# Orange-OpenSource/pyDcop

Measured on AMD Instinct MI355X. Metric: MaxSum iterations/sec on 100k-var random graph-coloring DCOP, higher is better.
Workload: dtype f64; 1 GPU; coloring_100k; n_vars=100000, n_factors=200000, n_edges=400000, domain=3, params=damping 0.5/both, stability 0.1, start leafs, parallelism=one GPU, 1 launch(es) per cycle, parity_checked=True, parity_test=tests/test_gpu_parity.py::test_north_star_100k_coloring

## Files before the change

### pydcop_amd/csrc/kernels.h

```cpp
#pragma once
#include <hip/hip_runtime.h>

#include <cmath>
#include <cstdint>
#include <cstring>
#include <type_traits>
#include <utility>

#include "layout.h"

namespace mxs {

constexpr int SAME_COUNT = 4;
#ifndef MXS_ASM_MIN
#define MXS_ASM_MIN 1
#endif
#ifndef SWEEP_MIN_WAVES
#define SWEEP_MIN_WAVES 4
#endif

#ifndef MXS_NT
#define MXS_NT 0
#endif
constexpr int NT_STREAMING = 9;
#define MXS_NT_FLAGS(NT)                                                                        \
    constexpr bool NT_IDX = ((NT) & 1) != 0, NT_PREV = ((NT) & 2) != 0, NT_GATHER = ((NT) & 4) != 0; \
    (void)NT_IDX, (void)NT_PREV, (void)NT_GATHER
template <bool NT, typename U>
__device__ __forceinline__ U ldp(const U* p) {
    if constexpr (NT) return __builtin_nontemporal_load(p);
    return *p;
}

template <typename F, int... I>
__device__ __forceinline__ void static_for_impl(F&& f, std::integer_sequence<int, I...>) {
    (f(std::integral_constant<int, I>{}), ...);
}
template <int N, typename F>
__device__ __forceinline__ void static_for(F&& f) {
    static_for_impl(f, std::make_integer_sequence<int, N>{});
}

constexpr int STAGE_BYTES_PER_WAVE = 64 * 2 * MAX_REG_D * 8;
__shared__ double g_stage[BLOCK / 64][STAGE_BYTES_PER_WAVE / 8];

struct Piece16 {
    unsigned int w[4];
};
typedef unsigned int v4u __attribute__((ext_vector_type(4)));
template <bool NT_STORE>
__device__ __forceinline__ void store_piece16(char* dst, const char* src) {
    if constexpr (NT_STORE) {
        __builtin_nontemporal_store(*(const v4u*)__builtin_assume_aligned(src, 16), (v4u*)__builtin_assume_aligned(dst, 16));
        return;
    }
    *(Piece16*)__builtin_assume_aligned(dst, 16) = *(const Piece16*)__builtin_assume_aligned(src, 16);
}
#ifndef MXS_NT_TIGHT
#define MXS_NT_TIGHT 1
#endif

template <typename T, int ELEMS, int NT = MXS_NT>
__device__ __forceinline__ void wave_store_linear(T* arr, int64_t wave_base, const T (&vals)[ELEMS]) {
    constexpr bool NT_STORE = (NT & 8) != 0;
    static_assert(64 * ELEMS * sizeof(T) % 16 == 0 && 64 * ELEMS * sizeof(T) <= STAGE_BYTES_PER_WAVE, "");
    if constexpr (ELEMS * sizeof(T) % 16 != 0) {
        const int w = (int)threadIdx.x >> 6, l = (int)threadIdx.x & 63;
        char* so = (char*)g_stage[w];
        __builtin_amdgcn_wave_barrier();
#pragma unroll
        for (int d = 0; d < ELEMS; ++d) ((T*)so)[l * ELEMS + d] = vals[d];
        __builtin_amdgcn_wave_barrier();
        char* out = (char*)(arr + wave_base);
        constexpr int BYTES = 64 * ELEMS * (int)sizeof(T), FULL = BYTES / 1024, REST = (BYTES % 1024) / 16;
#pragma unroll
        for (int k = 0; k < FULL; ++k) store_piece16<NT_STORE && MXS_NT_TIGHT>(out + k * 1024 + l * 16, so + k * 1024 + l * 16);
        if (REST > 0 && l < REST) store_piece16<NT_STORE && MXS_NT_TIGHT>(out + FULL * 1024 + l * 16, so + FULL * 1024 + l * 16);
        return;
    }
    const int w = (int)threadIdx.x >> 6, l = (int)threadIdx.x & 63;
    char* so = (char*)g_stage[w];
    __builtin_amdgcn_wave_barrier();
#pragma unroll
    for (int d = 0; d < ELEMS; ++d) ((T*)so)[l * ELEMS + d] = vals[d];
    __builtin_amdgcn_wave_barrier();
    char* out = (char*)(arr + wave_base);
    constexpr int PIECES = ELEMS * (int)sizeof(T) / 16;
#pragma unroll
    for (int k = 0; k < PIECES; ++k) store_piece16<NT_STORE>(out + k * 1024 + l * 16, so + k * 1024 + l * 16);
}

template <typename T>
struct SweepArgs {
    const T* v2f_old;
    T* v2f_new;
    const T* f2v_old;
    T* f2v_new;
    const T* tables;
    const uint8_t* ctables;
    int32_t tab_neg;
    const T* var_cost;
    uint8_t* cF;
    uint8_t* cV;
    const int32_t* edge_v2f;
    const int32_t* f2v_off;
    const int32_t* vrowptr;
    const int32_t* vslot_f2v;
    const int32_t* vslot_v2f;
    const int32_t* vell;
    const WaveMeta* vwave;
    const HubBlock* hub_blocks;
    const int32_t* vdom;
    const int64_t* vcost_off;
    const int32_t* init_idx;
    const FactorGen* fgen;
    const int32_t* edge_gen_factor;
    const int32_t* edge_dom;
    int32_t* sel;
    T* belief;
    T damping;
    T stability;
    int32_t damp_f;
    int32_t damp_v;
    int32_t start;
    int32_t start_mode;
    int32_t null_f2v;
    int64_t* timeline;
    uint32_t* halo_flags;
    uint32_t need_epoch;
    T* send_out;
    const int32_t* send_slot;
    int32_t n_peers;
    int32_t me;
    int32_t ghost_lo;
    const T* ghost_old;
    int32_t peer_first[MXS_MAX_PEERS];
    T* peer_dst[MXS_MAX_PEERS];
    int32_t n_classes;
    int32_t block_base[MAX_CLASSES];
    const ClassInfo* classes;
    const uint32_t* sched;
};

template <typename T>
__device__ __forceinline__ T pos_inf() {
    return (T)INFINITY;
}
__device__ __forceinline__ double absT(double x) { return fabs(x); }
__device__ __forceinline__ float absT(float x) { return fabsf(x); }

template <typename T>
__device__ __forceinline__ bool comp_match(T c, T prev_c, T stability) {
    if (prev_c != c) {
        const T delta = absT(prev_c - c);
        if (prev_c + c != (T)0) {
            if (!(((T)2 * delta / absT(prev_c + c)) < stability)) return false;
        } else {
            return false;
        }
    }
    return true;
}

template <typename T, int D>
__device__ __forceinline__ uint8_t damp_and_filter(T (&m)[D], const T (&prev)[D], uint8_t cnt,
                                                   bool damp_on, T damping, T stability) {
    if (cnt > 0 && damp_on) {
#pragma unroll
        for (int d = 0; d < D; ++d) m[d] = damping * prev[d] + ((T)1 - damping) * m[d];
    }
    bool match = cnt > 0;
#pragma unroll
    for (int d = 0; d < D; ++d) match = match && comp_match(m[d], prev[d], stability);
    if (!match) return 1;
    if (cnt < SAME_COUNT) return (uint8_t)(cnt + 1);
#pragma unroll
    for (int d = 0; d < D; ++d) m[d] = prev[d];
    return cnt;
}

template <typename T, int D>
struct Msg {
    static constexpr int H = half_stride(D, (int)sizeof(T));
    static constexpr int ALIGN = (H * (int)sizeof(T)) % 16 == 0 ? 16 : ((H * (int)sizeof(T)) % 8 == 0 ? 8 : 4);
    template <bool NT = false>
    static __device__ __forceinline__ void load(const T* p, T (&m)[D]) {
        const T* q = (const T*)__builtin_assume_aligned(p, ALIGN);
#pragma unroll
        for (int d = 0; d < D; ++d) m[d] = ldp<NT>(q + d);
    }
    static __device__ __forceinline__ void store(T* p, const T (&m)[D]) {
        T* q = (T*)__builtin_assume_aligned(p, ALIGN);
#pragma unroll
        for (int d = 0; d < H; ++d) q[d] = d < D ? m[d < D ? d : 0] : (T)0;
    }
    static __device__ __forceinline__ void load_sys(const T* p, T (&m)[D]) {
#pragma unroll
        for (int d = 0; d < D; ++d) m[d] = __hip_atomic_load(p + d, __ATOMIC_RELAXED, __HIP_MEMORY_SCOPE_SYSTEM);
    }
    static constexpr bool CNT_IN_MSG = H > D;
    template <bool NT = false>
    static __device__ __forceinline__ uint8_t load_c(const T* p, T (&m)[D]) {
        const T* q = (const T*)__builtin_assume_aligned(p, ALIGN);
#pragma unroll
        for (int d = 0; d < D; ++d) m[d] = ldp<NT>(q + d);
        return (uint8_t)(int)ldp<NT>(q + (D < H ? D : 0));
    }
    static __device__ __forceinline__ T padded(const T (&m)[D], uint8_t cnt, int d) {
        return d < D ? m[d < D ? d : 0] : (d == D ? (T)(int)cnt : (T)0);
    }
    static __device__ __forceinline__ void store_c(T* p, const T (&m)[D], uint8_t cnt) {
        T* q = (T*)__builtin_assume_aligned(p, ALIGN);
#pragma unroll
        for (int d = 0; d < H; ++d) q[d] = padded(m, cnt, d);
    }
};

template <typename T, int N, int NT = MXS_NT>
__device__ __forceinline__ void load_table(const SweepArgs<T>& a, const ClassInfo& ci, int j, T (&tab)[N]) {
    MXS_NT_FLAGS(NT);
    if (ci.tab_type == TAB_FULL) {
#pragma unroll
        for (int k = 0; k < N; ++k) tab[k] = ldp<NT_IDX>(a.tables + ci.tab_base + (int64_t)k * ci.count + j);
        return;
    }
    if (ci.tab_type == TAB_I8) {
        constexpr int REC = tab_record_bytes(N, 1);
        uint32_t w[REC / 4];
        const uint32_t* p = (const uint32_t*)__builtin_assume_aligned(
            a.ctables + ci.ctab_base + (int64_t)j * REC, REC >= 16 ? 16 : REC);
#pragma unroll
        for (int i = 0; i < REC / 4; ++i) w[i] = ldp<NT_IDX>(p + i);
#pragma unroll
        for (int k = 0; k < N; ++k) tab[k] = (T)(int)(int8_t)(uint8_t)(w[k >> 2] >> (8 * (k & 3)));
    } else if (ci.tab_type == TAB_I16) {
        constexpr int REC = tab_record_bytes(N, 2);
        uint32_t w[REC / 4];
        const uint32_t* p = (const uint32_t*)__builtin_assume_aligned(
            a.ctables + ci.ctab_base + (int64_t)j * REC, REC >= 16 ? 16 : REC);
#pragma unroll
        for (int i = 0; i < REC / 4; ++i) w[i] = ldp<NT_IDX>(p + i);
#pragma unroll
        for (int k = 0; k < N; ++k) tab[k] = (T)(int)(int16_t)(uint16_t)(w[k >> 1] >> (16 * (k & 1)));
    } else {
        constexpr int REC = tab_record_bytes(N, 4);
        uint32_t w[REC / 4];
        const uint32_t* p = (const uint32_t*)__builtin_assume_aligned(
            a.ctables + ci.ctab_base + (int64_t)j * REC, REC >= 16 ? 16 : REC);
#pragma unroll
        for (int i = 0; i < REC / 4; ++i) w[i] = ldp<NT_IDX>(p + i);
#pragma unroll
        for (int k = 0; k < N; ++k) {
            float f;
            __builtin_memcpy(&f, &w[k], 4);
            tab[k] = (T)f;
        }
    }
    if (a.tab_neg) {
#pragma unroll
        for (int k = 0; k < N; ++k) tab[k] = -tab[k];
    }
}

template <typename T, int D, int NT = MXS_NT>
__device__ __forceinline__ void factor_unary(const SweepArgs<T>& a, const ClassInfo& ci, int j) {
    MXS_NT_FLAGS(NT);
    constexpr int H = Msg<T, D>::H;
    const int64_t fo = ci.f2v_base + (int64_t)j * H;
    const int e = ci.edge_base + j;
    constexpr bool CIM = Msg<T, D>::CNT_IN_MSG;
    T out[D], prev[D], tab[D];
    uint8_t cn;
    if constexpr (CIM) cn = Msg<T, D>::template load_c<NT_PREV>(a.f2v_old + fo, prev);
    else {
        Msg<T, D>::template load<NT_PREV>(a.f2v_old + fo, prev);
        cn = a.cF[e];
    }
    load_table<T, D, NT>(a, ci, j, tab);
#pragma unroll
    for (int d = 0; d < D; ++d)
        out[d] = tab[d] + (T)0;
    uint8_t c = 0;
    if (!a.start)
        c = damp_and_filter<T, D>(out, prev, cn, a.damp_f != 0, a.damping, a.stability);
    if constexpr (CIM) {
        Msg<T, D>::store_c(a.f2v_new + fo, out, c);
    } else {
        Msg<T, D>::store(a.f2v_new + fo, out);
        a.cF[e] = c;
    }
}

template <typename T, int D, bool P2P = false, int NT = MXS_NT, bool CUT_HALF = true>
__device__ __forceinline__ void factor_binary(const SweepArgs<T>& a, const ClassInfo& ci, int j) {
    MXS_NT_FLAGS(NT);
    constexpr int H = Msg<T, D>::H;
    const int e = ci.edge_base + 2 * j;
    const int64_t fo0 = ci.f2v_base + (int64_t)j * H, fo1 = ci.f2v_base1 + (int64_t)j * H;
    constexpr bool CIM = Msg<T, D>::CNT_IN_MSG;
    const bool do0 = !CUT_HALF || ci.own_pos != 2, do1 = !CUT_HALF || ci.own_pos != 1;
    const int v0 = do1 ? ldp<NT_IDX>(a.edge_v2f + e) : 0, v1 = do0 ? ldp<NT_IDX>(a.edge_v2f + e + 1) : 0;
    uint8_t cn0 = 0, cn1 = 0;
    T m0[D], p0[D], m1[D], p1[D], tab[D * D];
#pragma unroll
    for (int d = 0; d < D; ++d) m0[d] = p0[d] = m1[d] = p1[d] = (T)0;
    if constexpr (CIM) {
        if (do0) cn0 = Msg<T, D>::template load_c<NT_PREV>(a.f2v_old + fo0, p0);
        if (do1) cn1 = Msg<T, D>::template load_c<NT_PREV>(a.f2v_old + fo1, p1);
    } else {
        if (do0) {
            cn0 = a.cF[e];
            Msg<T, D>::template load<NT_PREV>(a.f2v_old + fo0, p0);
        }
        if (do1) {
            cn1 = a.cF[e + 1];
            Msg<T, D>::template load<NT_PREV>(a.f2v_old + fo1, p1);
        }
    }
    load_table<T, D * D, NT>(a, ci, j, tab);
    if constexpr (P2P) {
        if (do1) {
            if (v0 >= a.ghost_lo) Msg<T, D>::load_sys(a.ghost_old + (v0 - a.ghost_lo), m0);
            else Msg<T, D>::load(a.v2f_old + v0, m0);
        }
        if (do0) {
            if (v1 >= a.ghost_lo) Msg<T, D>::load_sys(a.ghost_old + (v1 - a.ghost_lo), m1);
            else Msg<T, D>::load(a.v2f_old + v1, m1);
        }
    } else {
        if (do1) Msg<T, D>::template load<NT_GATHER>(a.v2f_old + v0, m0);
        if (do0) Msg<T, D>::template load<NT_GATHER>(a.v2f_old + v1, m1);
    }
    T o0[D], o1[D];
#pragma unroll
    for (int x = 0; x < D; ++x) {
        T best0 = pos_inf<T>(), best1 = pos_inf<T>();
#pragma unroll
        for (int y = 0; y < D; ++y) {
            const T c0 = tab[x * D + y] + ((T)0 + m1[y]);
            if (best0 > c0) best0 = c0;
            const T c1 = tab[y * D + x] + ((T)0 + m0[y]);
            if (best1 > c1) best1 = c1;
        }
        o0[x] = best0;
        o1[x] = best1;
    }
    uint8_t c0 = 0, c1 = 0;
    if (a.start) {
        const bool sends = a.start_mode == MXS_START_ALL;
#pragma unroll
        for (int d = 0; d < D; ++d) {
            o0[d] = sends ? o0[d] : (T)0;
            o1[d] = sends ? o1[d] : (T)0;
        }
    } else {
        c0 = damp_and_filter<T, D>(o0, p0, cn0, a.damp_f != 0, a.damping, a.stability);
        c1 = damp_and_filter<T, D>(o1, p1, cn1, a.damp_f != 0, a.damping, a.stability);
    }
    const int lw = (int)threadIdx.x & 63;
    if constexpr ((64 * H * sizeof(T)) % 16 == 0) {
        if ((j - lw + 63) < ci.count) {
            T full[H];
            if (do0) {
#pragma unroll
                for (int d = 0; d < H; ++d) full[d] = Msg<T, D>::padded(o0, CIM ? c0 : 0, d);
                wave_store_linear<T, H, NT>(a.f2v_new, fo0 - (int64_t)lw * H, full);
            }
            if (do1) {
#pragma unroll
                for (int d = 0; d < H; ++d) full[d] = Msg<T, D>::padded(o1, CIM ? c1 : 0, d);
                wave_store_linear<T, H, NT>(a.f2v_new, fo1 - (int64_t)lw * H, full);
            }
        } else {
            if (do0) Msg<T, D>::store_c(a.f2v_new + fo0, o0, CIM ? c0 : 0);
            if (do1) Msg<T, D>::store_c(a.f2v_new + fo1, o1, CIM ? c1 : 0);
        }
    } else {
        if (do0) Msg<T, D>::store_c(a.f2v_new + fo0, o0, CIM ? c0 : 0);
        if (do1) Msg<T, D>::store_c(a.f2v_new + fo1, o1, CIM ? c1 : 0);
    }
    if constexpr (!CIM) {
        if (do0) a.cF[e] = c0;
        if (do1) a.cF[e + 1] = c1;
    }
}

template <typename T>
__device__ __forceinline__ T factor_gen_value(const SweepArgs<T>& a, const FactorGen& fg, int pos,
                                              int d, int64_t others) {
    T best = pos_inf<T>();
    for (int64_t lin = 0; lin < others; ++lin) {
        int64_t rem = others, l = lin, t = 0;
        T sum_cost = (T)0;
        for (int i = 0; i < fg.arity; ++i) {
            const int e = fg.edge_base + i;
            const int Di = a.edge_dom[e];
            int digit;
            if (i == pos) {
                digit = d;
            } else {
                rem /= Di;
                digit = (int)(l / rem);
                l -= (int64_t)digit * rem;
                sum_cost += a.v2f_old[a.edge_v2f[e] + digit];
            }
            t = t * Di + digit;
        }
        const T cur = a.tables[fg.tab_off + t] + sum_cost;
        if (best > cur) best = cur;
    }
    return best;
}

template <typename T>
__device__ __forceinline__ void factor_generic(const SweepArgs<T>& a, const ClassInfo& ci, int j) {
    const int e = ci.edge_base + j;
    const FactorGen fg = a.fgen[a.edge_gen_factor[e]];
    const int pos = e - fg.edge_base;
    const int D = a.edge_dom[e];
    const T* prev = a.f2v_old + a.f2v_off[e];
    T* w = a.f2v_new + a.f2v_off[e];
    int64_t others = 1;
    for (int i = 0; i < fg.arity; ++i)
        if (i != pos) others *= a.edge_dom[fg.edge_base + i];
    if (a.start) {
        const bool sends = (fg.arity == 1 && a.start_mode != MXS_START_ALL) ||
                           a.start_mode == MXS_START_ALL;
        for (int d = 0; d < D; ++d) w[d] = sends ? factor_gen_value(a, fg, pos, d, others) : (T)0;
        a.cF[e] = 0;
        return;
    }
    const uint8_t cnt = a.cF[e];
    const bool damp = cnt > 0 && a.damp_f;
    bool match = cnt > 0;
    for (int d = 0; d < D; ++d) {
        T m = factor_gen_value(a, fg, pos, d, others);
        const T p = prev[d];
        if (damp) m = a.damping * p + ((T)1 - a.damping) * m;
        if (match) match = comp_match(m, p, a.stability);
        w[d] = m;
    }
    uint8_t out = 1;
    if (match) {
        if (cnt < SAME_COUNT) {
            out = (uint8_t)(cnt + 1);
        } else {
            out = cnt;
            for (int d = 0; d < D; ++d) w[d] = prev[d];
        }
    }
    a.cF[e] = out;
}

template <typename T, int D, bool P2P = false, int NT = MXS_NT>
__device__ __forceinline__ void variable_pack(const SweepArgs<T>& a, const ClassInfo& ci, int item) {
    MXS_NT_FLAGS(NT);
    constexpr int H = Msg<T, D>::H;
    const int lane_id = item + (int)threadIdx.x;
    if (lane_id >= ci.count) return;
    const int64_t pos = ci.ell_base + lane_id;
    const WaveMeta wm = a.vwave[__builtin_amdgcn_readfirstlane((int)(pos >> 6))];
    const uint32_t dn = (uint32_t)wm.deg_nv;
    const int deg = (int)(dn & 255u), nv = (int)((dn >> 8) & 255u);
    const int l = (int)threadIdx.x & 63;
    const int var = (int)(((uint32_t)l * (dn >> 16)) >> 15);
    const int k = l - var * deg;
    const bool has = var < nv;
    const int v = wm.first_var + (has ? var : 0);
    const int32_t slot = ldp<NT_IDX>(a.vell + pos);
    const int32_t send_at = a.send_slot != nullptr ? a.send_slot[pos] : -1;
    constexpr bool CIM = Msg<T, D>::CNT_IN_MSG;
    T pv[D], in[D], c[D], b[D], m[D];
    const int64_t vo = ci.v2f_base + (int64_t)lane_id * H;
    uint8_t cnt;
    if constexpr (CIM) cnt = Msg<T, D>::template load_c<NT_PREV>(a.v2f_old + vo, pv);
    else {
        cnt = a.cV[ci.cv_base + lane_id];
        Msg<T, D>::template load<NT_PREV>(a.v2f_old + vo, pv);
    }
    Msg<T, D>::template load<NT_GATHER>(a.f2v_old + (has ? slot : a.null_f2v), in);
#pragma unroll
    for (int d = 0; d < D; ++d) c[d] = a.var_cost[ci.cost_base + (int64_t)(v - ci.first) * D + d];
    int init = -1;
    if (a.start) init = a.init_idx[v];
    const int seg = l - (has ? k : 0);
    T sum_cost = (T)0;
#pragma unroll
    for (int d = 0; d < D; ++d) {
        T bd = c[d], md = c[d];
        for (int kk = 0; kk < deg; ++kk) {
            const T x = __shfl(in[d], seg + kk, 64);
            bd += x;
            if (kk != k) {
                sum_cost += x;
                md += x;
            }
        }
        b[d] = bd;
        m[d] = md;
    }
    int best = 0;
    T best_c = b[0];
#pragma unroll
    for (int d = 1; d < D; ++d)
        if (b[d] < best_c) {
            best = d;
            best_c = b[d];
        }
    if (init >= 0) {
        best = init;
        best_c = (T)0;
    }
    if (has && k == 0) {
        a.sel[v] = best;
        a.belief[v] = best_c;
    }
    const T avg = sum_cost / (T)D;
#pragma unroll
    for (int d = 0; d < D; ++d) m[d] = m[d] - avg;
    uint8_t co = 0;
    if (a.start) {
        const bool sends = (deg == 1 && a.start_mode == MXS_START_LEAFS) ||
                           a.start_mode != MXS_START_LEAFS;
#pragma unroll
        for (int d = 0; d < D; ++d) m[d] = sends ? m[d] : (T)0;
    } else {
        co = damp_and_filter<T, D>(m, pv, cnt, a.damp_v != 0, a.damping, a.stability);
    }
    if (!has) {
        co = 0;
#pragma unroll
        for (int d = 0; d < D; ++d) m[d] = (T)0;
    }
    if (send_at >= 0) {
        T* dst = a.send_out + (int64_t)send_at * H;
        if constexpr (P2P) {
            T* base = a.peer_dst[0];
            int first = a.peer_first[0];
#pragma unroll
            for (int q = 1; q < MXS_MAX_PEERS; ++q) {
                const bool ge = send_at >= a.peer_first[q];
                base = ge ? a.peer_dst[q] : base;
                first = ge ? a.peer_first[q] : first;
            }
            dst = base + (int64_t)(send_at - first) * H;
        }
        Msg<T, D>::store_c(dst, m, CIM ? co : 0);
    }
    if constexpr ((64 * H * sizeof(T)) % 16 == 0) {
        T full[H];
#pragma unroll
        for (int d = 0; d < H; ++d) full[d] = Msg<T, D>::padded(m, CIM ? co : 0, d);
        wave_store_linear<T, H, NT>(a.v2f_new, vo - (int64_t)l * H, full);
    } else {
        Msg<T, D>::store(a.v2f_new + vo, m);
    }
    if constexpr (!CIM) a.cV[ci.cv_base + lane_id] = co;
}

constexpr int PACK8_D = 8;
template <typename T>
__device__ __forceinline__ void variable_pack8_block(const SweepArgs<T>& a, const ClassInfo& ci, int block) {
    constexpr int H = PACK8_D;
    static_assert(half_stride(5, (int)sizeof(T)) == H && half_stride(8, (int)sizeof(T)) == H, "records of 5..8 values are 8 elements long");
    const int lane_id = block * BLOCK + (int)threadIdx.x;
    if (lane_id >= ci.count) return;
    const int64_t pos = ci.ell_base + lane_id;
    const WaveMeta wm = a.vwave[__builtin_amdgcn_readfirstlane((int)(pos >> 6))];
    const uint32_t dn = (uint32_t)wm.deg_nv;
    const int deg = (int)(dn & 255u), nv = (int)((dn >> 8) & 255u);
    const int l = (int)threadIdx.x & 63;
    const int var = (int)(((uint32_t)l * (dn >> 16)) >> 15);
    const int k = l - var * deg;
    const bool has = var < nv;
    const int v = wm.first_var + (has ? var : 0);
    const int32_t slot = a.vell[pos];
    const int D = ci.uni_D ? ci.uni_D : a.vdom[v];
    const int64_t vo = ci.v2f_base + (int64_t)lane_id * H;
    const uint8_t cnt = a.cV[ci.cv_base + lane_id];
    T pv[H], in[H], c[H], m[H];
    Msg<T, H>::load(a.v2f_old + vo, pv);
    Msg<T, H>::load(a.f2v_old + (has ? slot : a.null_f2v), in);
    const T* cp = a.var_cost + (ci.uni_D ? ci.cost_base + (int64_t)(v - ci.first) * ci.uni_D : a.vcost_off[v]);
#pragma unroll
    for (int d = 0; d < H; ++d) {
        c[d] = d < D ? cp[d < D ? d : 0] : (T)0;
        in[d] = d < D ? in[d] : (T)0;
    }
    int init = -1;
    if (a.start) init = a.init_idx[v];
    const int seg = l - (has ? k : 0);
    T sum_cost = (T)0, best_c = (T)0;
    int best = 0;
    const int DU = ci.uni_D ? ci.uni_D : H;
    static_for<H>([&](auto dc) __attribute__((always_inline)) {
        constexpr int d = decltype(dc)::value;
        T bd = c[d], md = c[d];
        if (d < DU) {
            for (int kk = 0; kk < deg; ++kk) {
                const T x = __shfl(in[d], seg + kk, 64);
                bd += x;
                if (kk != k) {
                    sum_cost += x;
                    md += x;
                }
            }
        }
        m[d] = md;
        if (d == 0 || (d < D && bd < best_c)) {
            best = d;
            best_c = bd;
        }
    });
    if (init >= 0) {
        best = init;
        best_c = (T)0;
    }
    if (has && k == 0) {
        a.sel[v] = best;
        a.belief[v] = best_c;
    }
    const T avg = sum_cost / (T)D;
#pragma unroll
    for (int d = 0; d < H; ++d) m[d] = m[d] - avg;
    uint8_t co = 0;
    if (a.start) {
        const bool sends = (deg == 1 && a.start_mode == MXS_START_LEAFS) || a.start_mode != MXS_START_LEAFS;
#pragma unroll
        for (int d = 0; d < H; ++d) m[d] = sends ? m[d] : (T)0;
    } else {
        if (cnt > 0 && a.damp_v) {
#pragma unroll
            for (int d = 0; d < H; ++d) m[d] = a.damping * pv[d] + ((T)1 - a.damping) * m[d];
        }
        bool match = cnt > 0;
#pragma unroll
        for (int d = 0; d < H; ++d) match = match && (d >= D || comp_match(m[d], pv[d], a.stability));
        if (!match) {
            co = 1;
        } else if (cnt < SAME_COUNT) {
            co = (uint8_t)(cnt + 1);
        } else {
            co = cnt;
#pragma unroll
            for (int d = 0; d < H; ++d) m[d] = pv[d];
        }
    }
#pragma unroll
    for (int d = 0; d < H; ++d) m[d] = (has && d < D) ? m[d] : (T)0;
    if (!has) co = 0;
    wave_store_linear<T, H>(a.v2f_new, vo - (int64_t)l * H, m);
    a.cV[ci.cv_base + lane_id] = co;
}
template <typename T>
__global__ void __launch_bounds__(BLOCK) k_variable_pack8(SweepArgs<T> a, const ClassInfo* __restrict__ cls) {
    const ClassInfo ci = cls[0];
    variable_pack8_block<T>(a, ci, (int)blockIdx.x);
}

template <typename T>
__device__ __forceinline__ void variable_generic(const SweepArgs<T>& a, const ClassInfo& ci, int j) {
    if (ci.start_only && !a.start) return;
    const int v = ci.first + j;
    const int D = a.vdom[v];
    const int k0 = a.vrowptr[v], k1 = a.vrowptr[v + 1];
    const int deg = k1 - k0;
    const T* c = a.var_cost + a.vcost_off[v];
    int best = 0;
    T best_c = (T)0;
    for (int d = 0; d < D; ++d) {
        T b = c[d];
        for (int k = k0; k < k1; ++k) b += a.f2v_old[a.vslot_f2v[k] + d];
        if (d == 0 || b < best_c) {
            best = d;
            best_c = b;
        }
    }
    if (a.start && a.init_idx[v] >= 0) {
        best = a.init_idx[v];
        best_c = (T)0;
    }
    a.sel[v] = best;
    a.belief[v] = best_c;
    const bool start_sends = (deg == 1 && a.start_mode == MXS_START_LEAFS) ||
                             a.start_mode != MXS_START_LEAFS;
    for (int ko = k0; ko < k1; ++ko) {
        const T* prev = a.v2f_old + a.vslot_v2f[ko];
        T* w = a.v2f_new + a.vslot_v2f[ko];
        T sum_cost = (T)0;
        for (int d = 0; d < D; ++d)
            for (int k = k0; k < k1; ++k)
                if (k != ko) sum_cost += a.f2v_old[a.vslot_f2v[k] + d];
        const T avg = sum_cost / (T)D;
        const uint8_t cnt = a.start ? 0 : a.cV[ko];
        const bool damp = cnt > 0 && a.damp_v;
        bool match = cnt > 0;
        for (int d = 0; d < D; ++d) {
            T m = c[d];
            for (int k = k0; k < k1; ++k)
                if (k != ko) m += a.f2v_old[a.vslot_f2v[k] + d];
            m = m - avg;
            if (a.start) {
                w[d] = start_sends ? m : (T)0;
                continue;
            }
            const T p = prev[d];
            if (damp) m = a.damping * p + ((T)1 - a.damping) * m;
            if (match) match = comp_match(m, p, a.stability);
            w[d] = m;
        }
        uint8_t out = 1;
        if (a.start) {
            out = 0;
        } else if (match) {
            if (cnt < SAME_COUNT) {
                out = (uint8_t)(cnt + 1);
            } else {
                out = cnt;
                for (int d = 0; d < D; ++d) w[d] = prev[d];
            }
        }
        a.cV[ko] = out;
    }
}

__device__ __forceinline__ void lds_barrier() {
    __builtin_amdgcn_fence(__ATOMIC_RELEASE, "workgroup", "local");
    __builtin_amdgcn_s_barrier();
    __builtin_amdgcn_fence(__ATOMIC_ACQUIRE, "workgroup", "local");
}

template <typename T>
__device__ __forceinline__ void variable_hub(const SweepArgs<T>& a, const ClassInfo& ci, int item) {
    constexpr int R = HUB_LDS / BLOCK;
    static_assert(BLOCK == 128 * HUB_CW && (HUB_CW & (HUB_CW - 1)) == 0, "two waves (sum_cost, msg_costs) per 64 edges");
    __shared__ __attribute__((aligned(16))) T s_hub[HUB_LDS + 64];
    __shared__ T s_sum[HUB_EDGES];
    const int tid = (int)threadIdx.x, wave = tid >> 6, lane = tid & 63;
    const HubBlock hb = a.hub_blocks[ci.first + item];
    const int D = hb.D, k0 = hb.slot0, deg = hb.deg;
    const int grp = wave & (HUB_CW - 1);
    const bool msg_role = wave >= HUB_CW;
    const int ko_w = hb.ko0 + (grp << 6);
    const int ko = ko_w + lane;
    const bool wave_on = ko_w <= deg;
    const bool real = msg_role && wave_on && ko < deg, bel = msg_role && wave_on && ko == deg;
    const T* c = a.var_cost + hb.cost_off;
    const T nzero = (T)-0.0;
    if (wave_on) __builtin_amdgcn_s_setprio(3);
    const int NK = deg < HUB_TILE ? ((deg + 7) & ~7) : HUB_TILE, ROW = NK + 8;
    const int ND = HUB_LDS / ROW;
    const uint32_t magic = hb.magic;
    const int vo = a.vslot_v2f[k0 + (real ? ko : 0)];
    const uint8_t cnt = a.start ? 0 : a.cV[k0 + (real ? ko : 0)];
    T pre[R];
    auto request = [&](int d0, int kt) __attribute__((always_inline)) {
        int off[R];
#pragma unroll
        for (int r = 0; r < R; ++r) {
            const int e = tid + BLOCK * r;
            const int dd = (int)(((uint64_t)(uint32_t)e * magic) >> 32), p = e - dd * ROW;
            const int k = kt + p - 8;
            const bool is_x = dd < ND && d0 + dd < D && p >= 8 && k < deg;
            off[r] = a.vslot_f2v[k0 + (is_x ? k : 0)];
        }
#pragma unroll
        for (int r = 0; r < R; ++r) {
            const int e = tid + BLOCK * r;
            const int dd = (int)(((uint64_t)(uint32_t)e * magic) >> 32), p = e - dd * ROW;
            const int dc = d0 + dd, k = kt + p - 8;
            const bool row_ok = dd < ND && dc < D;
            const bool is_x = row_ok && p >= 8 && k < deg, is_c = row_ok && p == 0;
            const T* src = is_x ? a.f2v_old + (off[r] + dc) : c + (is_c ? dc : 0);
            pre[r] = *src;
        }
    };
    T mreg[4] = {(T)0, (T)0, (T)0, (T)0};
    const bool park = D > 4;
    T acc = (T)0, best_c = (T)0;
    int best = 0;
    int d0 = 0, kt = 0;
    request(0, 0);
    while (d0 < D) {
        lds_barrier();
#pragma unroll
        for (int r = 0; r < R; ++r) {
            const int e = tid + BLOCK * r;
            const int dd = (int)(((uint64_t)(uint32_t)e * magic) >> 32), p = e - dd * ROW;
            const bool row_ok = dd < ND && d0 + dd < D;
            s_hub[e] = (row_ok && (p == 0 || (p >= 8 && kt + p - 8 < deg))) ? pre[r] : nzero;
        }
        lds_barrier();
        const bool last_k = kt + NK >= deg;
        const int d0n = last_k ? d0 + ND : d0, ktn = last_k ? 0 : kt + NK;
        if (d0n < D) request(d0n, ktn);
        const int n = deg - kt < NK ? deg - kt : NK;
        auto walk = [&](auto msg_c) __attribute__((always_inline)) {
            constexpr bool MSG = decltype(msg_c)::value;
            for (int dd = 0; dd < ND && d0 + dd < D; ++dd) {
                const T* row = s_hub + dd * ROW;
                if (MSG && kt == 0) acc = row[0];
                auto fetch = [&](T (&x)[8], int kk) __attribute__((always_inline)) {
#pragma unroll
                    for (int u = 0; u < 8; ++u) x[u] = row[8 + kk + u];
                };
                auto consume = [&](T (&x)[8], int kk, auto sel) __attribute__((always_inline)) {
                    if constexpr (decltype(sel)::value) {
                        const int kabs = kt + kk;
#pragma unroll
                        for (int u = 0; u < 8; ++u) x[u] = (kabs + u == ko) ? nzero : x[u];
                    }
#pragma unroll
                    for (int u = 0; u < 8; ++u) acc += x[u];
                };
                auto run = [&](int k_lo, int k_hi, auto sel) __attribute__((always_inline)) {
                    if (k_lo >= k_hi) return;
                    T xa[8], xb[8], xc[8];
                    fetch(xa, k_lo);
                    fetch(xb, k_lo + 8);
                    int kk = k_lo;
                    for (; kk + 24 <= k_hi; kk += 24) {
                        fetch(xc, kk + 16);
                        consume(xa, kk, sel);
                        fetch(xa, kk + 24);
                        consume(xb, kk + 8, sel);
                        fetch(xb, kk + 32);
                        consume(xc, kk + 16, sel);
                    }
                    if (kk < k_hi) consume(xa, kk, sel);
                    if (kk + 8 < k_hi) consume(xb, kk + 8, sel);
                };
                const int n8 = (n + 7) & ~7;
                const int w_lo = ko_w - kt < 0 ? 0 : (ko_w - kt > n8 ? n8 : ((ko_w - kt) & ~7));
                const int w_hi = ko_w + 64 - kt < 0 ? 0 : (ko_w + 64 - kt > n8 ? n8 : ((ko_w + 64 - kt + 7) & ~7));
                run(0, w_lo, std::false_type{});
                run(w_lo, w_hi, std::true_type{});
                run(w_hi, n8, std::false_type{});
                if (MSG && last_k) {
                    const int d = d0 + dd;
                    if (park) {
                        if (real) a.v2f_new[vo + d] = acc;
                    } else {
#pragma unroll
                        for (int q = 0; q < 4; ++q) mreg[q] = d == q ? acc : mreg[q];
                    }
                    if (d == 0 || acc < best_c) {
                        best = d;
                        best_c = acc;
                    }
                }
            }
        };
        if (wave_on) {
            if (msg_role) walk(std::true_type{});
            else walk(std::false_type{});
        }
        d0 = d0n;
        kt = ktn;
    }
    if (!msg_role && wave_on) s_sum[(grp << 6) + lane] = acc;
    lds_barrier();
    if (bel) {
        const int v = hb.var;
        if (a.start && a.init_idx[v] >= 0) {
            best = a.init_idx[v];
            best_c = (T)0;
        }
        a.sel[v] = best;
        a.belief[v] = best_c;
    }
    if (!real) return;
    const T avg = s_sum[(grp << 6) + lane] / (T)D;
    const T* prev = a.v2f_old + vo;
    T* w = a.v2f_new + vo;
    const bool start_sends = (deg == 1 && a.start_mode == MXS_START_LEAFS) || a.start_mode != MXS_START_LEAFS;
    const bool damp = cnt > 0 && a.damp_v;
    bool match = cnt > 0;
    for (int dd = 0; dd < D; ++dd) {
        T mm = park ? w[dd] : (dd == 0 ? mreg[0] : dd == 1 ? mreg[1] : dd == 2 ? mreg[2] : mreg[3]);
        mm = mm - avg;
        if (a.start) {
            w[dd] = start_sends ? mm : (T)0;
            continue;
        }
        const T p = prev[dd];
        if (damp) mm = a.damping * p + ((T)1 - a.damping) * mm;
        if (match) match = comp_match(mm, p, a.stability);
        w[dd] = mm;
    }
    uint8_t out = 1;
    if (a.start) {
        out = 0;
    } else if (match) {
        if (cnt < SAME_COUNT) {
            out = (uint8_t)(cnt + 1);
        } else {
            out = cnt;
            for (int dd = 0; dd < D; ++dd) w[dd] = prev[dd];
        }
    }
    a.cV[k0 + ko] = out;
}

template <typename T, int D, bool P2P = false, int NT = MXS_NT, bool CUT_HALF = true>
__device__ __forceinline__ void sweep_d(const SweepArgs<T>& a, const ClassInfo& ci, int item) {
    if (ci.kind == K_V_PACK) {
        variable_pack<T, D, P2P, NT>(a, ci, item);
        return;
    }
    const int j = item + (int)threadIdx.x;
    if (j >= ci.count) return;
    if (ci.kind == K_F_BIN) factor_binary<T, D, P2P, NT, CUT_HALF>(a, ci, j);
    else if (ci.kind == K_F_UNARY) factor_unary<T, D, NT>(a, ci, j);
}

constexpr unsigned long long HALO_WAIT_TICKS = 500000000ull;
constexpr int HALO_ERR_WORD = 32;
__device__ __forceinline__ void wait_for_halo(uint32_t* flags, uint32_t need, int n_peers, int me) {
    if (threadIdx.x == 0) {
        const unsigned long long t0 = wall_clock64();
        const int n = n_peers > 0 ? n_peers : 1;
        for (int q = 0; q < n; ++q) {
            if (n_peers > 0 && q == me) continue;
            while (__hip_atomic_load(flags + q, __ATOMIC_RELAXED, __HIP_MEMORY_SCOPE_SYSTEM) < need &&
                   __hip_atomic_load(flags + HALO_ERR_WORD, __ATOMIC_RELAXED, __HIP_MEMORY_SCOPE_AGENT) == 0) {
                __builtin_amdgcn_s_sleep(64);
                if (wall_clock64() - t0 > HALO_WAIT_TICKS) {
                    atomicOr(flags + HALO_ERR_WORD, 1u);
                    break;
                }
            }
        }
        if (n_peers > 0) __builtin_amdgcn_fence(__ATOMIC_ACQUIRE, "");
    }
    __syncthreads();
    if (n_peers > 0) {
        __builtin_amdgcn_fence(__ATOMIC_ACQUIRE, "workgroup");
    } else {
        __builtin_amdgcn_fence(__ATOMIC_ACQUIRE, "agent");
    }
}

template <typename T, int DSEL, bool P2P = false, int NT = MXS_NT, bool SCHED = false, bool HUB = false>
__device__ __forceinline__ int sweep_block(const SweepArgs<T>& a) {
    int c = 0, blk = -1;
    if (SCHED || a.sched != nullptr) {
        const uint32_t s = a.sched[blockIdx.x];
        c = (int)(s >> 24);
        blk = (int)(s & 0xffffffu);
    } else {
#pragma unroll
        for (int i = 1; i < MAX_CLASSES; ++i) c += ((int)blockIdx.x >= a.block_base[i]) ? 1 : 0;
    }
    const ClassInfo ci = a.classes[c];
    const int item = (blk >= 0 ? blk : (int)blockIdx.x - ci.block_base) * ci.per_block;
    if (!SCHED && ci.wait_halo && a.halo_flags != nullptr) wait_for_halo(a.halo_flags, a.need_epoch, a.n_peers, a.me);
    if (HUB && ci.kind == K_V_HUB) {
        variable_hub<T>(a, ci, item);
        return ci.kind;
    }
    if (ci.kind == K_F_GEN || ci.kind == K_V_GEN) {
        const int j = item + (int)threadIdx.x;
        if (j >= ci.count) return ci.kind;
        if (ci.kind == K_F_GEN) factor_generic<T>(a, ci, j);
        else variable_generic<T>(a, ci, j);
        return ci.kind;
    }
    if (DSEL != 0) {
        sweep_d<T, (DSEL != 0 ? DSEL : 2), P2P, NT, !SCHED>(a, ci, item);
    } else {
        switch (ci.D) {
            case 2: sweep_d<T, 2, P2P, NT, !SCHED>(a, ci, item); break;
            case 3: sweep_d<T, 3, P2P, NT, !SCHED>(a, ci, item); break;
            case 4: sweep_d<T, 4, P2P, NT, !SCHED>(a, ci, item); break;
            default: break;
        }
    }
    return ci.kind;
}

#ifndef SWEEP_SGPRS
#define SWEEP_SGPRS 104
#endif
template <typename T, int DSEL, int NT = MXS_NT, bool SCHED = false>
__global__ void __launch_bounds__(BLOCK, SWEEP_MIN_WAVES) __attribute__((amdgpu_num_sgpr(SWEEP_SGPRS)))
k_sweep(SweepArgs<T> a) {
    sweep_block<T, DSEL, false, NT, SCHED>(a);
}
template <typename T, int NT = MXS_NT, bool SCHED = false>
__global__ void __launch_bounds__(BLOCK, SWEEP_MIN_WAVES) __attribute__((amdgpu_num_sgpr(80)))
k_sweep_d2(SweepArgs<T> a) {
    sweep_block<T, 2, false, NT, SCHED>(a);
}

template <typename T, int DSEL, int NT = MXS_NT, bool SCHED = false>
__global__ void __launch_bounds__(BLOCK, SWEEP_MIN_WAVES) k_sweep_hub(SweepArgs<T> a) {
    sweep_block<T, DSEL, false, NT, SCHED, true>(a);
}

template <typename T, int DSEL>
__global__ void __launch_bounds__(BLOCK, SWEEP_MIN_WAVES) k_sweep_p2p(SweepArgs<T> a) {
    sweep_block<T, DSEL, true, MXS_NT, false, true>(a);
}

template <typename T, int DSEL, bool HUB>
__device__ __forceinline__ void sweep_timeline(const SweepArgs<T>& a) {
    const int64_t t0 = (int64_t)wall_clock64();
    const int kind = sweep_block<T, DSEL, false, MXS_NT, false, HUB>(a);
    __builtin_amdgcn_s_waitcnt(0);
    const int64_t t1 = (int64_t)wall_clock64();
    if (threadIdx.x == 0) {
        a.timeline[3 * (int64_t)blockIdx.x + 0] = t0;
        a.timeline[3 * (int64_t)blockIdx.x + 1] = t1;
        a.timeline[3 * (int64_t)blockIdx.x + 2] = kind;
    }
}
template <typename T, int DSEL>
__global__ void __launch_bounds__(BLOCK, SWEEP_MIN_WAVES) k_sweep_timeline(SweepArgs<T> a) {
    sweep_timeline<T, DSEL, false>(a);
}
template <typename T, int DSEL>
__global__ void __launch_bounds__(BLOCK) k_sweep_timeline_hub(SweepArgs<T> a) {
    sweep_timeline<T, DSEL, true>(a);
}

constexpr int NARY_MAX_SUMD = 1024;
constexpr int NARY_MAX_R = 1024;
constexpr int NARY_MAX_NJ = NARY_MAX_R / BLOCK;
constexpr int NARY_MAX_ARITY = 6;

template <typename T>
struct OrdKey;
template <>
struct OrdKey<double> {
    typedef unsigned long long U;
    static __device__ __forceinline__ U enc(double x) {
        U b;
        memcpy(&b, &x, 8);
        return (b >> 63) ? ~b : (b | 0x8000000000000000ull);
    }
    static __device__ __forceinline__ double dec(U k) {
        const U b = (k >> 63) ? (k & 0x7fffffffffffffffull) : ~k;
        double x;
        memcpy(&x, &b, 8);
        return x;
    }
};
template <>
struct OrdKey<float> {
    typedef unsigned int U;
    static __device__ __forceinline__ U enc(float x) {
        U b;
        memcpy(&b, &x, 4);
        return (b >> 31) ? ~b : (b | 0x80000000u);
    }
    static __device__ __forceinline__ float dec(U k) {
        const U b = (k >> 31) ? (k & 0x7fffffffu) : ~k;
        float x;
        memcpy(&x, &b, 4);
        return x;
    }
};

template <typename T>
__device__ __forceinline__ T wave_min(T x) {
#pragma unroll
    for (int s = 32; s > 0; s >>= 1) {
        const T y = __shfl(x, (int)((threadIdx.x & 63) ^ s), 64);
        x = y < x ? y : x;
    }
    return x;
}

__device__ __forceinline__ double min2(double x, double y) {
#if defined(__HIP_DEVICE_COMPILE__) && MXS_ASM_MIN
    double r;
    asm("v_min_f64 %0, %1, %2" : "=v"(r) : "v"(x), "v"(y));
    return r;
#else
    return __builtin_fmin(x, y);
#endif
}
__device__ __forceinline__ float min2(float x, float y) { return __builtin_fminf(x, y); }

template <int CTRL, int ROW_MASK>
__device__ __forceinline__ double dpp_mov(double x) {
    int lo = __double2loint(x), hi = __double2hiint(x);
    lo = __builtin_amdgcn_update_dpp(lo, lo, CTRL, ROW_MASK, 0xf, false);
    hi = __builtin_amdgcn_update_dpp(hi, hi, CTRL, ROW_MASK, 0xf, false);
    return __hiloint2double(hi, lo);
}
template <int CTRL, int ROW_MASK>
__device__ __forceinline__ float dpp_mov(float x) {
    int b = __float_as_int(x);
    b = __builtin_amdgcn_update_dpp(b, b, CTRL, ROW_MASK, 0xf, false);
    return __int_as_float(b);
}
typedef unsigned int swap2u __attribute__((ext_vector_type(2)));
template <bool W32, bool SECOND>
__device__ __forceinline__ unsigned int swap_word(unsigned int w) {
    const swap2u r = W32 ? __builtin_amdgcn_permlane32_swap(w, w, false, false)
                         : __builtin_amdgcn_permlane16_swap(w, w, false, false);
    return SECOND ? r[1] : r[0];
}
template <bool W32, bool SECOND>
__device__ __forceinline__ double swap_val(double x) {
    const unsigned int lo = swap_word<W32, SECOND>((unsigned int)__double2loint(x));
    const unsigned int hi = swap_word<W32, SECOND>((unsigned int)__double2hiint(x));
    return __hiloint2double((int)hi, (int)lo);
}
template <bool W32, bool SECOND>
__device__ __forceinline__ float swap_val(float x) {
    return __int_as_float((int)swap_word<W32, SECOND>((unsigned int)__float_as_int(x)));
}
template <typename T> __device__ __forceinline__ T swap16_lo(T x) { return swap_val<false, false>(x); }
template <typename T> __device__ __forceinline__ T swap16_hi(T x) { return swap_val<false, true>(x); }
template <typename T> __device__ __forceinline__ T swap32_lo(T x) { return swap_val<true, false>(x); }
template <typename T> __device__ __forceinline__ T swap32_hi(T x) { return swap_val<true, true>(x); }
template <typename T>
__device__ __forceinline__ T wave_min4(const T (&b)[4]) {
    const int l = (int)threadIdx.x & 63;
    const bool odd = (l & 1) != 0, hi = (l & 2) != 0;
    T k0 = odd ? b[2] : b[0], k1 = odd ? b[3] : b[1];
    const T s0 = odd ? b[0] : b[2], s1 = odd ? b[1] : b[3];
    k0 = min2(k0, dpp_mov<0xB1, 0xf>(s0));
    k1 = min2(k1, dpp_mov<0xB1, 0xf>(s1));
    T k = hi ? k1 : k0;
    const T s = hi ? k0 : k1;
    k = min2(k, dpp_mov<0x4E, 0xf>(s));
    k = min2(k, dpp_mov<0x124, 0xf>(k));
    k = min2(k, dpp_mov<0x128, 0xf>(k));
    k = min2(swap16_lo(k), swap16_hi(k));
    k = min2(swap32_lo(k), swap32_hi(k));
    return k;
}

constexpr int NARY_UNR = 4;

template <typename T, int A, int NJ, bool MASKED, bool LS = false>
__device__ __forceinline__ void nary_batch(const T (&tv)[NARY_UNR][NJ], int d0, int D0, const T* s_m0,
                                           const T (&ms)[NJ][A], const T (&s0)[NJ], const bool (&live)[NJ],
                                           T (&acc)[NJ][A], typename OrdKey<T>::U* s_key0) {
    T best0[NARY_UNR];
#pragma unroll
    for (int u = 0; u < NARY_UNR; ++u) {
        if (MASKED && d0 + u >= D0) {
            best0[u] = pos_inf<T>();
            continue;
        }
        const T m0 = s_m0[(!MASKED || d0 + u < D0) ? d0 + u : 0];
        const T a0 = m0;
        T b0 = pos_inf<T>();
        const T sp1_shared = (LS && A == 3) ? a0 + ms[0][A - 1] : (T)0;
#pragma unroll
        for (int j = 0; j < NJ; ++j) {
            T t = tv[u][j];
            if (MASKED) t = (live[j] && d0 + u < D0) ? t : pos_inf<T>();
            b0 = min2(b0, t + s0[j]);
#pragma unroll
            for (int p = 1; p < A; ++p) {
                T sp = a0;
                if (LS && A == 3 && p == 1) {
                    sp = sp1_shared;
                } else {
#pragma unroll
                    for (int i = 1; i < A; ++i)
                        if (i != p) sp += ms[j][i];
                }
                acc[j][p] = min2(acc[j][p], t + sp);
            }
        }
        best0[u] = b0;
    }
    static_assert(NARY_UNR == 4, "wave_min4 reduces four values");
    const T m = wave_min4(best0);
    const int l = (int)threadIdx.x & 63;
    const int u = 2 * (l & 1) + ((l >> 1) & 1);
    if (l < 4 && (!MASKED || d0 + u < D0)) atomicMin(&s_key0[d0 + u], OrdKey<T>::enc(m));
}

__device__ __forceinline__ void nary_divmod(int x, int D, uint32_t magic, int& q, int& r) {
    q = D == 1 ? x : (int)(((uint64_t)(uint32_t)x * magic) >> 32);
    r = x - q * D;
}

template <int A, int NJ>
__device__ __forceinline__ void nary_digits(int tid, int NT, const int (&Dm)[A], const uint32_t (&mg)[A],
                                            const bool (&live)[NJ], int (&dig)[NJ][A]) {
    int step[A];
    int rem = tid, rs = NT;
#pragma unroll
    for (int i = A - 1; i >= 1; --i) {
        int q;
        nary_divmod(rem, Dm[i], mg[i], q, dig[0][i]);
        rem = q;
        nary_divmod(rs, Dm[i], mg[i], q, step[i]);
        rs = q;
    }
#pragma unroll
    for (int j = 1; j < NJ; ++j) {
        int carry = 0;
#pragma unroll
        for (int i = A - 1; i >= 1; --i) {
            const int x = dig[j - 1][i] + step[i] + carry;
            carry = x >= Dm[i] ? 1 : 0;
            dig[j][i] = x - (carry ? Dm[i] : 0);
        }
    }
#pragma unroll
    for (int j = 0; j < NJ; ++j)
#pragma unroll
        for (int i = 1; i < A; ++i) dig[j][i] = live[j] ? dig[j][i] : Dm[i] - 1;
}

template <typename T, typename TT>
__device__ __forceinline__ T nary_slot_entry_fwd(const uint32_t* w, int j) {
    if constexpr (sizeof(TT) == 1) return (T)(int)(int8_t)(uint8_t)(w[j >> 2] >> (8 * (j & 3)));
    else return (T)(int)(int16_t)(uint16_t)(w[j >> 1] >> (16 * (j & 1)));
}

template <typename T, int A, int NJ, bool MULTI = false, typename TT = T, bool NEG = false>
__global__ void __launch_bounds__(BLOCK) k_factor_nary(SweepArgs<T> a, const NaryDesc* descs, int cap) {
    static_assert(MULTI || (std::is_same<TT, T>::value && !NEG), "narrow row-major images: the multi-pass groups only");
    typedef typename OrdKey<T>::U U;
    constexpr int UNR = NARY_UNR;
    HIP_DYNAMIC_SHARED(unsigned long long, s_dyn)
    T* s_msg = (T*)s_dyn;
    U* s_key = (U*)(s_msg + cap);
    T* s_prev = (T*)(s_key + cap);
    __shared__ int s_nomatch[NARY_MAX_ARITY];
    __shared__ int s_cnt[NARY_MAX_ARITY];
    const NaryDesc fd = descs[blockIdx.x];
    const int tid = (int)threadIdx.x, NT = (int)blockDim.x;
    int Dm[A], off[A];
    uint32_t mg[A];
    int sumd = 0;
#pragma unroll
    for (int i = 0; i < A; ++i) {
        Dm[i] = fd.dom[i];
        mg[i] = fd.magic[i];
        off[i] = sumd;
        sumd += Dm[i];
    }
    int R = 1;
#pragma unroll
    for (int i = 1; i < A; ++i) R *= Dm[i];
    const int D0 = Dm[0];
    const TT* tab = std::is_same<TT, T>::value ? (const TT*)(a.tables + fd.tab_off) : (const TT*)(a.ctables + fd.tab_off);
    constexpr bool RUN = !std::is_same<TT, T>::value;
    auto entry = [&](int64_t k) __attribute__((always_inline)) {
        if constexpr (!RUN) return tab[k];
        else {
            const T v = (T)(int)tab[k];
            return NEG ? -v : v;
        }
    };
    constexpr int RWD = RUN ? (NJ * (int)sizeof(TT) + 3) / 4 : 1;
    struct RowT { T v[NJ]; };
    struct RowW { uint32_t w[RWD]; };
    typedef typename std::conditional<RUN, RowW, RowT>::type Row;
    auto load_row = [&](int64_t row, const int (&qcl)[NJ], Row& out) __attribute__((always_inline)) {
        if constexpr (RUN) {
            __builtin_memcpy(out.w, (const uint8_t*)tab + (row + qcl[0]) * (int64_t)sizeof(TT), NJ * sizeof(TT));
        } else {
#pragma unroll
            for (int j = 0; j < NJ; ++j) out.v[j] = entry(row + qcl[j]);
        }
    };
    auto unpack = [&](const Row (&r)[UNR], T (&tv)[UNR][NJ]) __attribute__((always_inline)) {
#pragma unroll
        for (int u = 0; u < UNR; ++u)
#pragma unroll
            for (int j = 0; j < NJ; ++j) {
                if constexpr (RUN) {
                    const T v = nary_slot_entry_fwd<T, TT>(r[u].w, j);
                    tv[u][j] = NEG ? -v : v;
                } else {
                    tv[u][j] = r[u].v[j];
                }
            }
    };
    const int n_full = D0 / UNR;
    const int n_pass = MULTI ? (R + NJ * NT - 1) / (NJ * NT) : 1;
    for (int ps = 0; ps < n_pass; ++ps) {
    const int qb = ps * (NJ * NT);
    int qc[NJ];
    bool live[NJ];
#pragma unroll
    for (int j = 0; j < NJ; ++j) {
        const int q = RUN ? qb + tid * NJ + j : qb + tid + j * NT;
        live[j] = q < R;
        qc[j] = live[j] ? q : R - 1;
    }
    if (RUN && ps > 0 && qb + (tid & ~63) * NJ >= R) continue;
    Row cur[UNR];
    if (n_full > 0) {
#pragma unroll
        for (int u = 0; u < UNR; ++u) load_row((int64_t)u * R, qc, cur[u]);
    }
    if (ps == 0) {
#pragma unroll
    for (int i = 0; i < A; ++i) {
        const int vo = fd.v2f_off[i];
        for (int d = tid; d < Dm[i]; d += NT) {
            const T x = a.v2f_old[vo + d];
            s_msg[off[i] + d] = i == 0 ? (T)0 + x : x;
            s_key[off[i] + d] = OrdKey<T>::enc(pos_inf<T>());
        }
    }
    if (tid < NARY_MAX_ARITY) s_nomatch[tid] = 0;
    __syncthreads();
    }
    T ms[NJ][A], acc[NJ][A], s0[NJ];
    int dig[NJ][A];
    nary_digits<A, NJ>(RUN ? qb + tid * NJ : qb + tid, RUN ? 1 : NT, Dm, mg, live, dig);
#pragma unroll
    for (int j = 0; j < NJ; ++j) {
#pragma unroll
        for (int i = A - 1; i >= 1; --i) {
            ms[j][i] = s_msg[off[i] + dig[j][i]];
            acc[j][i] = pos_inf<T>();
        }
        T s = (T)0;
#pragma unroll
        for (int i = 1; i < A; ++i) s += ms[j][i];
        s0[j] = s;
    }
    const bool all_live = MULTI ? qb + NJ * NT <= R : R == NJ * NT;
    for (int b = 0; b < n_full; ++b) {
        const int d0 = b * UNR;
        Row nxt[UNR];
        if (b + 1 < n_full) {
#pragma unroll
            for (int u = 0; u < UNR; ++u) load_row((int64_t)(d0 + UNR + u) * R, qc, nxt[u]);
        } else {
#pragma unroll
            for (int u = 0; u < UNR; ++u) {
                if constexpr (RUN) {
#pragma unroll
                    for (int x = 0; x < RWD; ++x) nxt[u].w[x] = 0u;
                } else {
#pragma unroll
                    for (int j = 0; j < NJ; ++j) nxt[u].v[j] = pos_inf<T>();
                }
            }
        }
        T tv[UNR][NJ];
        unpack(cur, tv);
        if (all_live) nary_batch<T, A, NJ, false>(tv, d0, D0, s_msg + off[0], ms, s0, live, acc, s_key + off[0]);
        else nary_batch<T, A, NJ, true>(tv, d0, D0, s_msg + off[0], ms, s0, live, acc, s_key + off[0]);
#pragma unroll
        for (int u = 0; u < UNR; ++u) cur[u] = nxt[u];
    }
    if (n_full * UNR < D0) {
        const int d0 = n_full * UNR;
#pragma unroll
        for (int u = 0; u < UNR; ++u) load_row((int64_t)(d0 + u < D0 ? d0 + u : D0 - 1) * R, qc, cur[u]);
        T tv[UNR][NJ];
        unpack(cur, tv);
        nary_batch<T, A, NJ, true>(tv, d0, D0, s_msg + off[0], ms, s0, live, acc, s_key + off[0]);
    }
#pragma unroll
    for (int j = 0; j < NJ; ++j)
        if (live[j]) {
#pragma unroll
            for (int p = 1; p < A; ++p) atomicMin(&s_key[off[p] + dig[j][p]], OrdKey<T>::enc(acc[j][p]));
        }
    }
    __syncthreads();
    for (int idx = tid; idx < sumd; idx += NT) {
        int i = 0, off_i = 0, fo_i = fd.f2v_off[0];
#pragma unroll
        for (int ii = 1; ii < A; ++ii)
            if (idx >= off[ii]) {
                i = ii;
                off_i = off[ii];
                fo_i = fd.f2v_off[ii];
            }
        const int d = idx - off_i;
        T m = OrdKey<T>::dec(s_key[idx]);
        if (a.start) {
            s_msg[idx] = a.start_mode == MXS_START_ALL ? m : (T)0;
            continue;
        }
        const T p = a.f2v_old[fo_i + d];
        const int cnt = a.cF[fd.edge_base + i];
// ... 662 lines not shown
```

Before: 57070 iterations/s.

## Replace division-based stability test, stage variable sums in LDS, use min2 in factor

Adds a division-free send-rule test that compares 2|Δ| against stability·|sum| using guard bands, and falls back to the exact division only in ambiguous cases. Variable-pack belief sums now go through a per-wave staging buffer and chunked unrolled reads instead of one shuffle per neighbour. The factor min loop uses the v_min_f64 helper, which is moved earlier in the file. These target the f64 division cost, cross-lane shuffle latency and compare/select overhead, at the cost of extra LDS traffic, wave barriers and the risk of subtle parity drift in edge cases.

```diff
diff --git a/pydcop_amd/csrc/kernels.h b/pydcop_amd/csrc/kernels.h
--- a/pydcop_amd/csrc/kernels.h
+++ b/pydcop_amd/csrc/kernels.h
@@ -8,6 +8,7 @@
 #include <utility>
 
 #include "layout.h"
+#include "send_rule.h"
 
 namespace mxs {
 
@@ -149,18 +150,17 @@
 __device__ __forceinline__ double absT(double x) { return fabs(x); }
 __device__ __forceinline__ float absT(float x) { return fabsf(x); }
 
-template <typename T>
-__device__ __forceinline__ bool comp_match(T c, T prev_c, T stability) {
-    if (prev_c != c) {
-        const T delta = absT(prev_c - c);
-        if (prev_c + c != (T)0) {
-            if (!(((T)2 * delta / absT(prev_c + c)) < stability)) return false;
-        } else {
-            return false;
-        }
-    }
-    return true;
-}
+__device__ __forceinline__ double min2(double x, double y) {
+#if defined(__HIP_DEVICE_COMPILE__) && MXS_ASM_MIN
+    double r;
+    asm("v_min_f64 %0, %1, %2" : "=v"(r) : "v"(x), "v"(y));
+    return r;
+#else
+    return __builtin_fmin(x, y);
+#endif
+}
+__device__ __forceinline__ float min2(float x, float y) { return __builtin_fminf(x, y); }
+
 
 template <typename T, int D>
 __device__ __forceinline__ uint8_t damp_and_filter(T (&m)[D], const T (&prev)[D], uint8_t cnt,
@@ -169,9 +169,7 @@
 #pragma unroll
         for (int d = 0; d < D; ++d) m[d] = damping * prev[d] + ((T)1 - damping) * m[d];
     }
-    bool match = cnt > 0;
-#pragma unroll
-    for (int d = 0; d < D; ++d) match = match && comp_match(m[d], prev[d], stability);
+    const bool match = (cnt > 0) & msg_match<T, D>(m, prev, stability);
     if (!match) return 1;
     if (cnt < SAME_COUNT) return (uint8_t)(cnt + 1);
 #pragma unroll
@@ -337,10 +335,8 @@
         T best0 = pos_inf<T>(), best1 = pos_inf<T>();
 #pragma unroll
         for (int y = 0; y < D; ++y) {
-            const T c0 = tab[x * D + y] + ((T)0 + m1[y]);
-            if (best0 > c0) best0 = c0;
-            const T c1 = tab[y * D + x] + ((T)0 + m0[y]);
-            if (best1 > c1) best1 = c1;
+            best0 = min2(best0, tab[x * D + y] + ((T)0 + m1[y]));
+            best1 = min2(best1, tab[y * D + x] + ((T)0 + m0[y]));
         }
         o0[x] = best0;
         o1[x] = best1;
@@ -450,6 +446,52 @@
         }
     }
     a.cF[e] = out;
+}
+
+#ifndef MXS_SUM_CHUNK
+#define MXS_SUM_CHUNK 4
+#endif
+
+template <typename T, int D, int N>
+__device__ __forceinline__ void sum_chunk(const T* p, int own, T& bd, T& md, T& sum_cost) {
+    T x[N];
+#pragma unroll
+    for (int j = 0; j < N; ++j) x[j] = p[j * D];
+#pragma unroll
+    for (int j = 0; j < N; ++j) {
+        bd += x[j];
+        const T others = j == own ? (T)-0.0 : x[j];
+        sum_cost += others;
+        md += others;
+    }
+}
+
+template <typename T, int D>
+__device__ __forceinline__ void pack_sums(const T (&in)[D], const T (&c)[D], int seg, int k, int deg, T (&b)[D],
+                                          T (&m)[D], T& sum_cost) {
+    constexpr int C = MXS_SUM_CHUNK;
+    static_assert(64 * D * sizeof(T) <= STAGE_BYTES_PER_WAVE, "a wave's gathered records fit its staging area");
+    const int w = (int)threadIdx.x >> 6, l = (int)threadIdx.x & 63;
+    T* st = (T*)g_stage[w];
+    __builtin_amdgcn_wave_barrier();
+#pragma unroll
+    for (int d = 0; d < D; ++d) st[l * D + d] = in[d];
+    __builtin_amdgcn_wave_barrier();
+    const T* first = st + seg * D;
+    sum_cost = (T)0;
+    static_for<D>([&](auto dc) {
+        constexpr int d = decltype(dc)::value;
+        T bd = c[d], md = c[d];
+        const T* p = first + d;
+        int own = k, left = deg;
+        for (; left >= C; left -= C, own -= C, p += C * D) sum_chunk<T, D, C>(p, own, bd, md, sum_cost);
+        static_for<C - 1>([&](auto nc) {
+            constexpr int N = decltype(nc)::value + 1;
+            if (left == N) sum_chunk<T, D, N>(p, own, bd, md, sum_cost);
+        });
+        b[d] = bd;
+        m[d] = md;
+    });
 }
 
 template <typename T, int D, bool P2P = false, int NT = MXS_NT>
@@ -484,21 +526,25 @@
     int init = -1;
     if (a.start) init = a.init_idx[v];
     const int seg = l - (has ? k : 0);
-    T sum_cost = (T)0;
+    T sum_cost;
+#if MXS_SWEEP_SKIP & 1
+    sum_cost = (T)0;
 #pragma unroll
     for (int d = 0; d < D; ++d) {
         T bd = c[d], md = c[d];
         for (int kk = 0; kk < deg; ++kk) {
-            const T x = __shfl(in[d], seg + kk, 64);
-            bd += x;
+            bd += in[d];
             if (kk != k) {
-                sum_cost += x;
-                md += x;
+                sum_cost += in[d];
+                md += in[d];
             }
         }
         b[d] = bd;
         m[d] = md;
     }
+#else
+    pack_sums<T, D>(in, c, has ? seg : 0, k, deg, b, m, sum_cost);
+#endif
     int best = 0;
     T best_c = b[0];
 #pragma unroll
@@ -1071,17 +1117,6 @@
     }
     return x;
 }
-
-__device__ __forceinline__ double min2(double x, double y) {
-#if defined(__HIP_DEVICE_COMPILE__) && MXS_ASM_MIN
-    double r;
-    asm("v_min_f64 %0, %1, %2" : "=v"(r) : "v"(x), "v"(y));
-    return r;
-#else
-    return __builtin_fmin(x, y);
-#endif
-}
-__device__ __forceinline__ float min2(float x, float y) { return __builtin_fminf(x, y); }
 
 template <int CTRL, int ROW_MASK>
 __device__ __forceinline__ double dpp_mov(double x) {
diff --git a/pydcop_amd/csrc/send_rule.h b/pydcop_amd/csrc/send_rule.h
--- /dev/null
+++ b/pydcop_amd/csrc/send_rule.h
@@ -0,0 +1,96 @@
+#pragma once
+
+#ifndef MXS_HD
+#if defined(__HIPCC__)
+#define MXS_HD __host__ __device__ __forceinline__
+#else
+#define MXS_HD inline
+#endif
+#endif
+
+#ifndef MXS_SWEEP_SKIP
+#define MXS_SWEEP_SKIP 0
+#endif
+
+namespace mxs {
+
+MXS_HD double sr_abs(double x) { return __builtin_fabs(x); }
+MXS_HD float sr_abs(float x) { return __builtin_fabsf(x); }
+
+template <typename T>
+MXS_HD bool comp_match_div(T c, T prev_c, T stability) {
+    if (prev_c != c) {
+        const T delta = sr_abs(prev_c - c);
+        if (prev_c + c != (T)0) {
+            if (!(((T)2 * delta / sr_abs(prev_c + c)) < stability)) return false;
+        } else {
+            return false;
+        }
+    }
+    return true;
+}
+
+template <typename T>
+struct SendRuleBand;
+template <>
+struct SendRuleBand<double> {
+    static constexpr double LO = 1.0 - 0x1p-50, HI = 1.0 + 0x1p-50, STAB_MIN = 0x1p-1021;
+};
+template <>
+struct SendRuleBand<float> {
+    static constexpr float LO = 1.0f - 0x1p-21f, HI = 1.0f + 0x1p-21f, STAB_MIN = 0x1p-125f;
+};
+
+template <typename T>
+struct SendRuleEdges {
+    T lo, hi;
+    bool safe;
+};
+template <typename T>
+MXS_HD SendRuleEdges<T> send_rule_edges(T stability) {
+    using B = SendRuleBand<T>;
+    return {stability * B::LO, stability * B::HI, stability >= B::STAB_MIN};
+}
+
+template <typename T>
+MXS_HD void quotient_below_fast(T a, T s, const SendRuleEdges<T>& e, bool& yes, bool& no) {
+    const T lo = e.lo * s, hi = e.hi * s;
+#if MXS_SWEEP_SKIP & 2
+    yes = a < lo, no = !yes;
+    return;
+#endif
+    const bool safe = e.safe & (bool)__builtin_isnormal(lo);
+    yes = safe & (a < lo);
+    no = safe & (a > hi);
+}
+template <typename T>
+MXS_HD void comp_match_fast(T c, T prev_c, const SendRuleEdges<T>& e, bool& yes, bool& no) {
+    quotient_below_fast((T)2 * sr_abs(prev_c - c), sr_abs(prev_c + c), e, yes, no);
+}
+
+template <typename T>
+MXS_HD bool comp_match(T c, T prev_c, T stability) {
+    bool yes, no;
+    comp_match_fast(c, prev_c, send_rule_edges(stability), yes, no);
+    if (__builtin_expect(!(yes | no), 0)) return comp_match_div(c, prev_c, stability);
+    return yes;
+}
+
+template <typename T, int D>
+MXS_HD bool msg_match(const T (&m)[D], const T (&prev)[D], T stability) {
+    const SendRuleEdges<T> e = send_rule_edges(stability);
+    bool all_yes = true, any_no = false;
+    for (int d = 0; d < D; ++d) {
+        bool yes, no;
+        comp_match_fast(m[d], prev[d], e, yes, no);
+        all_yes &= yes;
+        any_no |= no;
+    }
+    if (__builtin_expect(!(all_yes | any_no), 0)) {
+        all_yes = true;
+        for (int d = 0; d < D; ++d) all_yes &= comp_match_div(m[d], prev[d], stability);
+    }
+    return all_yes;
+}
+
+}
```

New measurement: 59270 iterations/s (median of 6 runs). +3.9%, better.
